# CameronDiao/MolCLR

Hardware: AMD Instinct MI355X
Metric: contrastive pre-train molecules/sec at batch 512, 1/2/4/8 MI355X; HBM GB/s on scatter_add (higher is better)
Workload: dtype f32; 1 GPU; c2: GIN 5x300 feat 512, batch 512/GPU, 10-50 atom graphs; model=gin 5x300 feat 512, global_batch=512, per_gpu_batch=512, mean_nodes_per_view=15278, mean_edges_per_view=25094, parallelism=dp1, views=one paired encoder pass, per-view BatchNorm statistics, augment=host: pre-built resident batch pairs

## Files before the change

molclr_amd/csrc/gemm.hip:

```cpp
#include "mfma.h"

#include <stdlib.h>

#include <type_traits>

namespace {

using namespace molclr;

constexpr int LDK = BK + 4;
constexpr int RPAD = 4;

template <bool KMAJOR, int ROWS>
struct Image {
  static constexpr int FLOATS = KMAJOR ? BK * (ROWS + RPAD) : ROWS * LDK;
};

template <bool KMAJOR, int ROWS, int T>
struct Stager {
  static constexpr int ITEMS = ROWS * BK / 4;
  static constexpr int PER_THREAD = (ITEMS + T - 1) / T;
  float4 r[PER_THREAD];
  uint32_t ok;

// ... 425 lines not shown
      }
    }
  };

  const int nsteps = kt_end - kt_beg;
  auto kof = [&](int step) { return (int64_t)(kt_beg + step) * BK; };
  constexpr int CSN = CS == 1 ? SA::PER : CS == 2 ? SB::PER : 1;
  float4 cs[CSN];
#pragma unroll
  for (int j = 0; j < CSN; ++j) cs[j] = make_float4(0.f, 0.f, 0.f, 0.f);
  if (nsteps > 0) {
    sa0.load(kof(0), K, ta);
    sb0.load(kof(0), K, tb);
    if (nsteps > 1) {
      sa1.load(kof(1), K, ta);
      sb1.load(kof(1), K, tb);
    }
    if constexpr (CS) sa0.colsum_add(cs, ta);
    sa0.store(buf0, ta);
    sb0.store(buf0 + AI, tb);
    __syncthreads();
  }
  int i = 0;
  for (; i + 2 <= nsteps; i += 2) {
    if (i + 2 < nsteps) {
      sa0.load(kof(i + 2), K, ta);
      sb0.load(kof(i + 2), K, tb);
    }
    compute(buf0);
    if constexpr (CS) sa1.colsum_add(cs, ta);
    sa1.store(buf1, ta);
    sb1.store(buf1 + AI, tb);
    __syncthreads();
    if (i + 3 < nsteps) {
      sa1.load(kof(i + 3), K, ta);
      sb1.load(kof(i + 3), K, tb);
    }
    compute(buf1);
    if constexpr (CS) {
      if (i + 2 < nsteps) sa0.colsum_add(cs, ta);
    }
    sa0.store(buf0, ta);
    sb0.store(buf0 + AI, tb);
    __syncthreads();
  }
  if (i < nsteps) compute(buf0);

  if constexpr (CS) {
    if (n0 == 0 && colsum != nullptr) {
      constexpr int RB = BM / 4;
      float4 v = cs[0];
#pragma unroll
      for (int j = 1; j < CSN; ++j) v = f4add(v, cs[j]);
      __syncthreads();
      float4* red = reinterpret_cast<float4*>(lds);
      red[tid] = v;
      __syncthreads();
      if (tid < RB) {
        float4 t4 = red[tid];
        for (int q = 1; q < T / RB; ++q) t4 = f4add(t4, red[tid + q * RB]);
        const float e[4] = {t4.x, t4.y, t4.z, t4.w};
        float* o = SPLIT ? colsum + (int64_t)blockIdx.y * M : colsum;
        for (int j = 0; j < 4; ++j) {
          const int64_t m = m0 + 4 * tid + j;
          if (m < M) o[m] = (!SPLIT && accumulate) ? o[m] + e[j] : e[j];
        }
      }
    }
  }

  float* Cout = SPLIT ? C + (int64_t)blockIdx.y * M * N : C;
  const int64_t ldo = SPLIT ? N : ldc;
  constexpr int WR = 32 * TM, WC = 32 * TN;
  static_assert(4 * WR * WC * (int)sizeof(float) <= (int)sizeof(lds), "epilogue tile > LDS");
  const bool vec = ((ldo & 3) == 0) && ((reinterpret_cast<uintptr_t>(Cout) & 15) == 0) &&
                   (SPLIT || EPI != MOLCLR_EPI_RELU_MASK ||
                    (((ldaux & 3) == 0) && (reinterpret_cast<uintptr_t>(aux) & 15) == 0)) &&
                   (SPLIT || (EPI != MOLCLR_EPI_BIAS && EPI != MOLCLR_EPI_BIAS_RELU) ||
                    (reinterpret_cast<uintptr_t>(bias) & 15) == 0);
  if (vec) {
    __syncthreads();
    float* tw = reinterpret_cast<float*>(lds) + wave * WR * WC;
#pragma unroll
    for (int a = 0; a < TM; ++a)
#pragma unroll
      for (int b = 0; b < TN; ++b)
#pragma unroll
        for (int r = 0; r < 16; ++r)
          tw[(a * 32 + (r & 3) + 8 * (r >> 2) + 4 * lh) * WC + b * 32 + li] =
              acc[a][b][r] + acl[a][b][r];
    __syncthreads();
    constexpr int C4 = WC / 4;
    const int64_t mw = m0 + wm * WR, nw = n0 + wn * WC;
#pragma unroll
    for (int it = 0; it < WR * C4 / 64; ++it) {
      const int idx = it * 64 + lane;
      const int row = idx / C4, c4 = idx - row * C4;
      const int64_t m = mw + row, n = nw + 4 * c4;
      if (m >= M || n >= N) continue;
      float4 v = *reinterpret_cast<const float4*>(tw + row * WC + 4 * c4);
      float* o = Cout + m * ldo + n;
      if (n + 4 <= N) {
        if (!SPLIT) {
          if (EPI == MOLCLR_EPI_BIAS || EPI == MOLCLR_EPI_BIAS_RELU) {
            const float4 bv = *reinterpret_cast<const float4*>(bias + n);
            v = f4add(v, bv);
            if (EPI == MOLCLR_EPI_BIAS_RELU)
              v = make_float4(fmaxf(v.x, 0.f), fmaxf(v.y, 0.f), fmaxf(v.z, 0.f), fmaxf(v.w, 0.f));
          }
          if (EPI == MOLCLR_EPI_RELU_MASK) {
            const float4 x = *reinterpret_cast<const float4*>(aux + m * ldaux + n);
            v = make_float4(x.x > 0.f ? v.x : 0.f, x.y > 0.f ? v.y : 0.f, x.z > 0.f ? v.z : 0.f,
                            x.w > 0.f ? v.w : 0.f);
          }
          if (accumulate) v = f4add(v, *reinterpret_cast<const float4*>(o));
        }
        *reinterpret_cast<float4*>(o) = v;
      } else {
        const float e[4] = {v.x, v.y, v.z, v.w};
        for (int j = 0; j < 4 && n + j < N; ++j) {
          float x = e[j];
          if (!SPLIT) {
            if (EPI == MOLCLR_EPI_BIAS) x = x + bias[n + j];
            if (EPI == MOLCLR_EPI_BIAS_RELU) x = fmaxf(x + bias[n + j], 0.f);
            if (EPI == MOLCLR_EPI_RELU_MASK) x = aux[m * ldaux + n + j] > 0.f ? x : 0.f;
            if (accumulate) x += o[j];
          }
          o[j] = x;
        }
      }
    }
    return;
  }
#pragma unroll
  for (int b = 0; b < TN; ++b) {
    const int64_t n = n0 + wn * TN * 32 + b * 32 + li;
    if (n >= N) continue;
    float bv = 0.f;
    if (!SPLIT && (EPI == MOLCLR_EPI_BIAS || EPI == MOLCLR_EPI_BIAS_RELU)) bv = bias[n];
#pragma unroll
    for (int a = 0; a < TM; ++a) {
#pragma unroll
      for (int r = 0; r < 16; ++r) {
        const int64_t m = m0 + wm * TM * 32 + a * 32 + (r & 3) + 8 * (r >> 2) + 4 * lh;
        if (m >= M) continue;
        float v = acc[a][b][r] + acl[a][b][r];
        if (!SPLIT) {
          if (EPI == MOLCLR_EPI_BIAS) v = v + bv;
          if (EPI == MOLCLR_EPI_BIAS_RELU) v = fmaxf(v + bv, 0.f);
          if (EPI == MOLCLR_EPI_RELU_MASK) v = aux[m * ldaux + n] > 0.f ? v : 0.f;
          if (accumulate) v += Cout[m * ldo + n];
        }
        Cout[m * ldo + n] = v;
      }
    }
  }
}

constexpr int kQ6Waves = 4;
constexpr int kQ6BM = 32 * kQ6Waves;
constexpr int64_t kQ6MaxK = 1024;

template <int BN, int T, int NP = 3>
struct QStageB {
  static constexpr int UNITS = NP * BN * 4;
  static constexpr int PER = (UNITS + T - 1) / T;
  u32x4 r[PER];
  int goff[PER];
  __device__ __forceinline__ void init(int64_t n0, int64_t npad, int64_t kp, int t) {
#pragma unroll
    for (int j = 0; j < PER; ++j) {
      const int u = t + j * T;
      const int pl = u / (BN * 4), rem = u % (BN * 4);
      int64_t row = n0 + (rem >> 2);
      row = row < npad ? row : npad - 1;
      goff[j] = (UNITS % T && u >= UNITS) ? 0 : (int)((pl * npad + row) * kp + 8 * (rem & 3));
    }
  }
  __device__ __forceinline__ void load(const uint16_t* __restrict__ Bp, int64_t k0, int t) {
#pragma unroll
    for (int j = 0; j < PER; ++j) {
      if (j == PER - 1 && UNITS % T && t + j * T >= UNITS) continue;
      r[j] = *reinterpret_cast<const u32x4*>(Bp + goff[j] + k0);
    }
  }
  __device__ __forceinline__ void store(uint16_t* __restrict__ img, int t) const {
#pragma unroll
    for (int j = 0; j < PER; ++j) {
      const int u = t + j * T;
      if (j == PER - 1 && UNITS % T && u >= UNITS) continue;
      const int pl = u / (BN * 4), rem = u % (BN * 4);
      *reinterpret_cast<u32x4*>(img + pl * BN * XK + xoff(rem >> 2, rem & 3)) = r[j];
    }
  }
};

template <int BN, int NP>
__device__ __forceinline__ void q6_dma_b(const uint16_t* __restrict__ Bp, int64_t n0, int64_t npad,
                                         int64_t kp, int64_t k0, uint16_t* img, int wm, int lane) {
  constexpr int RPB = BN / 16, CH = NP * RPB, PERW = (CH + kQ6Waves - 1) / kQ6Waves;
  static_assert(BN % 16 == 0, "q6 DMA: 16-row chunks");
#pragma unroll
  for (int qq = 0; qq < PERW; ++qq) {
    const int q = wm + kQ6Waves * qq;
    if (CH % kQ6Waves && q >= CH) break;
    const int pl = q / RPB, row = (q % RPB) * 16 + (lane >> 2), c = lane & 3;
    int64_t gr = n0 + row;
    gr = gr < npad ? gr : npad - 1;
    __builtin_amdgcn_global_load_lds(
        (gbl_as_ptr)(Bp + (pl * npad + gr) * kp + k0 + 8 * (c ^ ((row >> 2) & 3))),
        (lds_as_ptr)(img + (pl * BN + (q % RPB) * 16) * XK), 16, 0, 0);
  }
}

template <int TN, int EPI, int KG, bool MASK, int H3 = 0>
__global__ __launch_bounds__(64 * kQ6Waves * KG) __attribute__((amdgpu_waves_per_eu(2))) void k_gemm_q6(
    const float* __restrict__ A, const uint16_t* __restrict__ Bp, float* __restrict__ C,
    int64_t M, int64_t N, int64_t K, int64_t lda, int64_t kp, int64_t npad, int64_t ldc,
    const float* __restrict__ bias, const float* __restrict__ aux, int64_t ldaux,
    int accumulate, const float* __restrict__ amax, const float* __restrict__ bmax,
    float* __restrict__ cmax, float* __restrict__ crow, float* __restrict__ amax_out,
    int arow_parts, uint32_t* __restrict__ bits_out, const uint32_t* __restrict__ bits_in,
    int64_t bits_ld) {
  constexpr int T = 64 * kQ6Waves;
  constexpr int BN = 32 * TN;
  constexpr int NP = H3 ? 2 : 3;
  constexpr int BI = NP * BN * XK;
  constexpr int EPI_ELEMS = kQ6Waves * 32 * 32 * 2;
  constexpr int L0 = KG == 1 ? (BI > EPI_ELEMS ? BI : EPI_ELEMS) : KG * 2 * BI;
  static_assert(KG == 1 || (kQ6Waves * 32 * BN * (int)sizeof(float) <=
                            KG * 2 * BI * (int)sizeof(uint16_t)),
                "group sums exceed the LDS images");
  __shared__ __attribute__((aligned(16))) uint16_t lds[L0];
  __shared__ __attribute__((aligned(16))) uint16_t lds_b1[KG == 1 ? BI : 8];

  const int tid = threadIdx.x;
  const int lane = tid & 63;
  const int wave = __builtin_amdgcn_readfirstlane(tid >> 6);
  const int grp = wave / kQ6Waves, wm = wave % kQ6Waves, gt = tid - grp * T;
  const int li = lane & 31, lh = lane >> 5;

  const int ntn = (int)((N + BN - 1) / BN);
  const int ntm = (int)((M + kQ6BM - 1) / kQ6BM);
  const int tile = xcd_remap(blockIdx.x, ntm * ntn);
  const int64_t m0 = (int64_t)(tile / ntn) * kQ6BM;
  const int64_t n0 = (int64_t)(tile % ntn) * BN;

  constexpr bool HAS_BIAS = EPI == MOLCLR_EPI_BIAS || EPI == MOLCLR_EPI_BIAS_RELU;
  constexpr int BVN = HAS_BIAS ? TN : 1, MWN = EPI == MOLCLR_EPI_RELU_MASK ? TN : 1;
  float4 bvq[BVN];
  uint32_t mwq[MWN][4];
  if (grp == 0) {
    const int c4l = lane & 7;
    if constexpr (HAS_BIAS) {
#pragma unroll
      for (int b = 0; b < TN; ++b) {
        const int64_t n = n0 + 32 * b + 4 * c4l;
        bvq[b] = (n + 4 <= N && (reinterpret_cast<uintptr_t>(bias) & 15) == 0)
                     ? *reinterpret_cast<const float4*>(bias + n) : f4zero();
      }
    }
    if constexpr (EPI == MOLCLR_EPI_RELU_MASK) {
      if (bits_in != nullptr) {
#pragma unroll
        for (int b = 0; b < TN; ++b)
#pragma unroll
          for (int it = 0; it < 4; ++it) {
            int64_t m = m0 + 32 * wm + 8 * it + (lane >> 3);
            m = m < M ? m : M - 1;
            int64_t nb = n0 + 32 * b;
            nb = nb < N ? nb : 0;
            mwq[b][it] = bits_in[(nb >> 5) * bits_ld + m];
          }
      }
    }
  }

  int64_t arow_i = m0 + 32 * wm + li;
  arow_i = arow_i < M ? arow_i : M - 1;
  const float* __restrict__ arow = A + arow_i * lda;
  const int nsteps = (int)(kp / BK);
  const int rounds = (nsteps + KG - 1) / KG;
  auto kb = [&](int r) {
    const int st = grp + KG * r;
    return (int64_t)(st < nsteps ? st : nsteps - 1) * BK;
  };
  auto load_a = [&](int r, float4(&v)[4]) {
    r = r < rounds ? r : rounds - 1;
    const int64_t k = (int64_t)(grp + KG * r) * BK + 16 * lh;
#pragma unroll
    for (int j = 0; j < 4; ++j) {
      int64_t kj = k + 4 * j;
      if constexpr (MASK) kj = kj < K - 4 ? kj : K - 4;
      v[j] = *reinterpret_cast<const float4*>(arow + kj);
    }
  };

  f32x16 acc[TN];
#pragma unroll
  for (int b = 0; b < TN; ++b)
#pragma unroll
    for (int r = 0; r < 16; ++r) acc[b][r] = 0.f;

  int sha = 0;
  if constexpr (H3 == 1) sha = h3_shift(amax);
  if constexpr (H3 == 2) {
// ... 2079 lines not shown
                         a.K, a.lda, a.ldb, npad, a.ldc, a.bias, a.aux, a.ldaux, a.accumulate,
                         a.amax, a.bmax, a.cmax, a.crow, a.amax_out, a.arow_parts, a.bits_out,
                         a.bits_in, a.bits_ld, ntn, groups);
  else if (wv == 16)
    molclr::launch_timed(molclr::kTimeGemm, (k_gemm_bsn<EPI, H3, 19, false, 16, 64>),
                         dim3((unsigned)(ntn * groups)), dim3(1024), 0, s, a.A, a.Bp, a.C, a.M, a.N,
                         a.K, a.lda, a.ldb, npad, a.ldc, a.bias, a.aux, a.ldaux, a.accumulate,
                         a.amax, a.bmax, a.cmax, a.crow, a.amax_out, a.arow_parts, a.bits_out,
                         a.bits_in, a.bits_ld, ntn, groups);
  else
    molclr::launch_timed(molclr::kTimeGemm, (k_gemm_bsn<EPI, H3, 19, false, 12, 64>),
                         dim3((unsigned)(ntn * groups)), dim3(768), 0, s, a.A, a.Bp, a.C, a.M, a.N,
                         a.K, a.lda, a.ldb, npad, a.ldc, a.bias, a.aux, a.ldaux, a.accumulate,
                         a.amax, a.bmax, a.cmax, a.crow, a.amax_out, a.arow_parts, a.bits_out,
                         a.bits_in, a.bits_ld, ntn, groups);
}
template <int H3>
int dispatch_bs64(int epi, const Args& a, int64_t npad, hipStream_t s) {
  switch (epi) {
    case MOLCLR_EPI_NONE: launch_bs64<MOLCLR_EPI_NONE, H3>(a, npad, s); return 0;
    case MOLCLR_EPI_BIAS: launch_bs64<MOLCLR_EPI_BIAS, H3>(a, npad, s); return 0;
    case MOLCLR_EPI_BIAS_RELU: launch_bs64<MOLCLR_EPI_BIAS_RELU, H3>(a, npad, s); return 0;
    case MOLCLR_EPI_RELU_MASK: launch_bs64<MOLCLR_EPI_RELU_MASK, H3>(a, npad, s); return 0;
    default: return -1;
  }
}
int64_t crow_parts(int64_t N) { return N > 320 ? (N + kBN - 1) / kBN : q6_col_tiles(N); }

int run_q6(const Args& a, int64_t npad, int epi, hipStream_t s, int h3 = 0) {
  if (h3 != 0 && use_bs(a, npad, epi, h3)) {
    const int rc = h3 == 2 ? dispatch_bs<2>(epi, a, npad, s) : dispatch_bs<1>(epi, a, npad, s);
    if (rc) {
      molclr::set_error("gemm_f32_h3: no bs kernel for epilogue %d", epi);
      return MOLCLR_ERR_UNSUPPORTED;
    }
    MOLCLR_LAUNCHED();
    return MOLCLR_OK;
  }
  if (h3 != 0 && use_bs64(a, npad, epi, h3)) {
    const int rc = h3 == 2 ? dispatch_bs64<2>(epi, a, npad, s) : dispatch_bs64<1>(epi, a, npad, s);
    if (rc) {
      molclr::set_error("gemm_f32_h3: no bs64 kernel for epilogue %d", epi);
      return MOLCLR_ERR_UNSUPPORTED;
    }
    MOLCLR_LAUNCHED();
    return MOLCLR_OK;
  }
  if (g_bs_force >= 2) {
    molclr::set_error("gemm_f32_h3_impl: the bs kernel does not take this product");
    return MOLCLR_ERR_UNSUPPORTED;
  }
  if (a.crow != nullptr && crow_parts(a.N) > q6_col_tiles(a.N)) {
    const int64_t w = q6_col_tiles(a.N);
    const hipError_t e = molclr::zero_async(a.crow + w * a.M,
                                            (size_t)(crow_parts(a.N) - w) * a.M * sizeof(float), s);
    if (e != hipSuccess) return (int)e;
  }
  const int rc = h3 == 2   ? dispatch_q6_tn<2>(epi, a, npad, s)
                 : h3 == 1 ? dispatch_q6_tn<1>(epi, a, npad, s)
                           : dispatch_q6_tn<0>(epi, a, npad, s);
  if (rc) {
    molclr::set_error("gemm_f32_bplanes: no q6 kernel for epilogue %d", epi);
    return MOLCLR_ERR_UNSUPPORTED;
  }
  MOLCLR_LAUNCHED();
  return MOLCLR_OK;
}

struct W6Plan {
  int tn, splits, kps, kg;
  int64_t ntiles;
};
W6Plan w6_plan(int64_t M, int64_t N, int64_t K, int kg) {
  W6Plan p;
  p.tn = wide_tn(N);
  p.kg = kg;
  p.ntiles = ((M + kW6BM - 1) / kW6BM) * ((N + 32 * p.tn - 1) / (32 * p.tn));
  const int64_t nk = (K + BK - 1) / BK;
  int64_t s = (512 / p.kg) / p.ntiles;
  if (s > nk / (4 * p.kg)) s = nk / (4 * p.kg);
  if (s < 1) s = 1;
  p.kps = (int)((nk + s - 1) / s);
  p.splits = (int)((nk + p.kps - 1) / p.kps);
  return p;
}
bool w6_shape_ok(int64_t M, int64_t N, int64_t K) {
  return M % 4 == 0 && N % 4 == 0 && K >= 1024 && M * N < (1ll << 28);
}
size_t w6_ws_bytes(int64_t M, int64_t N, int64_t K, bool colsum) {
  size_t need = 0;
  for (int kg = 1; kg <= 2; ++kg)
    for (int tr = 0; tr < 2; ++tr) {
      const W6Plan p = tr ? w6_plan(N, M, K, kg) : w6_plan(M, N, K, kg);
      const size_t b = (size_t)p.splits * (M * N + (colsum ? M : 0)) * sizeof(float) + 256;
      need = b > need ? b : need;
    }
  return need;
}

template <int TN, int KG, bool H3>
void launch_w6_kg(const W6Plan& p, hipStream_t s, const float* A, const float* B, float* part,
                  int64_t M, int64_t N, int64_t K, int64_t lda, int64_t ldb, float* cs_part,
                  const float* amax, const float* bmax, bool cs_b) {
  const dim3 grid((unsigned)(p.ntiles * p.splits));
  if (cs_part && cs_b)
    molclr::launch_timed(molclr::kTimeGemm, (k_gemm_w6<TN, 2, KG, H3>), grid, dim3(256 * KG), 0,
                         s, A, B, part, M, N, K, lda, ldb, p.kps, p.splits, cs_part, amax, bmax);
  else if (cs_part)
    molclr::launch_timed(molclr::kTimeGemm, (k_gemm_w6<TN, 1, KG, H3>), grid, dim3(256 * KG), 0,
                         s, A, B, part, M, N, K, lda, ldb, p.kps, p.splits, cs_part, amax, bmax);
  else
    molclr::launch_timed(molclr::kTimeGemm, (k_gemm_w6<TN, 0, KG, H3>), grid, dim3(256 * KG),
                         0, s, A, B, part, M, N, K, lda, ldb, p.kps, p.splits, cs_part, amax, bmax);
}
template <int TN, bool H3>
void launch_w6(const W6Plan& p, hipStream_t s, const float* A, const float* B, float* part,
               int64_t M, int64_t N, int64_t K, int64_t lda, int64_t ldb, float* cs_part,
               const float* amax, const float* bmax, bool cs_b = false) {
  if (p.kg == 2)
    launch_w6_kg<TN, 2, H3>(p, s, A, B, part, M, N, K, lda, ldb, cs_part, amax, bmax, cs_b);
  else
    launch_w6_kg<TN, 1, H3>(p, s, A, B, part, M, N, K, lda, ldb, cs_part, amax, bmax, cs_b);
}

int run_w6(const float* A, const float* B, float* C, float* colsum, int64_t M, int64_t N,
           int64_t K, int64_t lda, int64_t ldb, int64_t ldc, int accumulate, void* ws,
           size_t ws_bytes, hipStream_t s, int kg = 2, const float* amax = nullptr,
           const float* bmax = nullptr) {
  const W6Plan p = w6_plan(M, N, K, kg);
  MOLCLR_REQUIRE_WS(ws_bytes, w6_ws_bytes(M, N, K, colsum != nullptr));
  float* part = static_cast<float*>(ws);
  float* cs_part = colsum ? part + (size_t)p.splits * M * N : nullptr;
  if (amax) {
    if (p.tn == 5) launch_w6<5, true>(p, s, A, B, part, M, N, K, lda, ldb, cs_part, amax, bmax);
    else if (p.tn == 4) launch_w6<4, true>(p, s, A, B, part, M, N, K, lda, ldb, cs_part, amax, bmax);
    else launch_w6<2, true>(p, s, A, B, part, M, N, K, lda, ldb, cs_part, amax, bmax);
  } else {
    if (p.tn == 5) launch_w6<5, false>(p, s, A, B, part, M, N, K, lda, ldb, cs_part, amax, bmax);
    else if (p.tn == 4) launch_w6<4, false>(p, s, A, B, part, M, N, K, lda, ldb, cs_part, amax, bmax);
    else launch_w6<2, false>(p, s, A, B, part, M, N, K, lda, ldb, cs_part, amax, bmax);
  }
  const float* no_f = nullptr;
  molclr::launch_timed(molclr::kTimeGemm, k_splitk_reduce<MOLCLR_EPI_NONE>,
                       dim3((unsigned)molclr::ceil_div(M * N, 256)), dim3(256), 0, s,
                       static_cast<const float*>(part), p.splits, M, N, C, ldc, no_f, no_f,
                       (int64_t)0, accumulate, static_cast<const float*>(cs_part), p.splits, colsum);
  MOLCLR_LAUNCHED();
  return MOLCLR_OK;
}

int64_t planes_npad(int64_t N) { return (N + kPlanesRowPad - 1) / kPlanesRowPad * kPlanesRowPad; }
int64_t planes_kp(int64_t K) { return (K + BK - 1) / BK * BK; }

int run_gemm(const Args& a0, int impl, bool bp, int a_kmajor, int b_kmajor, int epilogue,
             void* workspace, size_t workspace_bytes, hipStream_t s) {
  const int64_t M = a0.M, N = a0.N, K = a0.K;
  int64_t tiles = tiles_for(impl, M, N, a_kmajor, b_kmajor);
  MOLCLR_REQUIRE(tiles < (1ll << 31), "gemm_f32: too many tiles");
  int sp = pick_splits(impl, M, N, K, a_kmajor, b_kmajor);
  const size_t cs_floats = a0.colsum ? (size_t)M : 0;
  if (sp > 1 && workspace_bytes < (size_t)sp * (M * N + cs_floats) * sizeof(float)) sp = 1;
  Args a = a0;
  a.impl = impl;
  int rc;
  if (sp == 1) {
    rc = bp ? dispatch_bplanes<false>(impl, a_kmajor, epilogue, dim3((unsigned)tiles), s, a)
            : dispatch<false>(a_kmajor != 0, b_kmajor != 0, epilogue, dim3((unsigned)tiles), s, a);
  } else {
    int64_t nk = (K + BK - 1) / BK;
    int kps = (int)((nk + sp - 1) / sp);
    sp = (int)((nk + kps - 1) / kps);
    float* partial = (float*)workspace;
    float* cs_partial = a.colsum ? partial + (size_t)sp * M * N : nullptr;
    Args ap = a;
    ap.C = partial;
    ap.colsum = cs_partial;
    ap.ldc = N;
    ap.bias = nullptr;
    ap.aux = nullptr;
    ap.ldaux = 0;
    ap.kps = kps;
    ap.accumulate = 0;
    rc = bp ? dispatch_bplanes<true>(impl, a_kmajor, MOLCLR_EPI_NONE, dim3((unsigned)tiles, sp), s, ap)
            : dispatch<true>(a_kmajor != 0, b_kmajor != 0, MOLCLR_EPI_NONE,
                             dim3((unsigned)tiles, sp), s, ap);
    if (rc == 0) {
      dim3 g((unsigned)molclr::ceil_div(M * N, 256));
      float* C = a.C;
      const int64_t ldc = a.ldc, ldaux = a.ldaux;
      const float *bias = a.bias, *aux = a.aux;
      const int accumulate = a.accumulate;
      switch (epilogue) {
        case MOLCLR_EPI_NONE:
          molclr::launch_timed(molclr::kTimeGemm, k_splitk_reduce<MOLCLR_EPI_NONE>, g, dim3(256), 0, s,
                               partial, sp, M, N, C, ldc, bias, aux, ldaux, accumulate, cs_partial, sp, a.colsum);
          break;
        case MOLCLR_EPI_BIAS:
          molclr::launch_timed(molclr::kTimeGemm, k_splitk_reduce<MOLCLR_EPI_BIAS>, g, dim3(256), 0, s,
                               partial, sp, M, N, C, ldc, bias, aux, ldaux, accumulate, cs_partial, sp, a.colsum);
          break;
        case MOLCLR_EPI_BIAS_RELU:
          molclr::launch_timed(molclr::kTimeGemm, k_splitk_reduce<MOLCLR_EPI_BIAS_RELU>, g, dim3(256), 0,
                               s, partial, sp, M, N, C, ldc, bias, aux, ldaux, accumulate, cs_partial, sp, a.colsum);
          break;
        default:
          molclr::launch_timed(molclr::kTimeGemm, k_splitk_reduce<MOLCLR_EPI_RELU_MASK>, g, dim3(256), 0,
                               s, partial, sp, M, N, C, ldc, bias, aux, ldaux, accumulate, cs_partial, sp, a.colsum);
      }
    }
  }
  if (rc != 0) {
    molclr::set_error("gemm_f32: no kernel for this layout");
    return MOLCLR_ERR_UNSUPPORTED;
  }
  MOLCLR_LAUNCHED();
  return MOLCLR_OK;
}

}

void molclr_splitk_reduce_none(const float* partial, int splits, int64_t M, int64_t N, float* C,
                               int64_t ldc, int accumulate, const float* cs_partial,
                               int cs_splits, float* colsum, hipStream_t s) {
  const float* no_f = nullptr;
  molclr::launch_timed(molclr::kTimeGemm, k_splitk_reduce<MOLCLR_EPI_NONE>,
                       dim3((unsigned)molclr::ceil_div(M * N > M ? M * N : M, 256)), dim3(256), 0,
                       s, partial, splits, M, N, C, ldc, no_f, no_f, (int64_t)0, accumulate,
                       cs_partial, cs_splits, colsum);
}

MOLCLR_API size_t molclr_gemm_f32_workspace_bytes(int64_t M, int64_t N, int64_t K) {
  int sp = pick_splits(0, M, N, K);
  for (int impl = 5; impl <= 8; ++impl) {
    const int s2 = pick_splits(impl, M, N, K);
    sp = s2 > sp ? s2 : sp;
  }
  const int s3 = pick_splits(5, M, N, K, 1, 1);
  sp = s3 > sp ? s3 : sp;
  size_t need = sp > 1 ? (size_t)sp * M * N * sizeof(float) + 256 : 0;
  if (w6_shape_ok(M, N, K)) {
    const size_t w6 = w6_ws_bytes(M, N, K, false);
    need = w6 > need ? w6 : need;
  }
  return need;
}

MOLCLR_API int molclr_gemm_f32_impl(const float* A, const float* B, float* C, int64_t M, int64_t N,
                                    int64_t K, int64_t lda, int64_t ldb, int64_t ldc, int a_kmajor,
                                    int b_kmajor, int epilogue_flags, const float* bias,
                                    const float* aux, int64_t ldaux, void* workspace,
                                    size_t workspace_bytes, molclr_stream_t stream, int impl_req) {
  const int accumulate = (epilogue_flags & MOLCLR_EPI_ACCUMULATE) ? 1 : 0;
  const int epilogue = epilogue_flags & ~MOLCLR_EPI_ACCUMULATE;
  MOLCLR_REQUIRE(impl_req == -1 || impl_req == 0 || impl_req == 5 || impl_req == 6,
                 "gemm_f32: impl %d (-1 automatic, 0, 5, 6)", impl_req);
  MOLCLR_REQUIRE(M >= 0 && N >= 0 && K >= 0, "gemm_f32: negative size");
  MOLCLR_REQUIRE(epilogue >= MOLCLR_EPI_NONE && epilogue <= MOLCLR_EPI_RELU_MASK,
                 "gemm_f32: bad epilogue %d", epilogue);
  MOLCLR_REQUIRE((epilogue != MOLCLR_EPI_BIAS && epilogue != MOLCLR_EPI_BIAS_RELU) || bias,
                 "gemm_f32: bias epilogue needs bias");
  MOLCLR_REQUIRE(epilogue != MOLCLR_EPI_RELU_MASK || aux, "gemm_f32: relu-mask epilogue needs aux");
  MOLCLR_REQUIRE(a_kmajor || (K % 4 == 0 && lda % 4 == 0),
                 "gemm_f32: A with K contiguous needs K (%lld) and lda multiples of 4", (long long)K);
  MOLCLR_REQUIRE(b_kmajor || (K % 4 == 0 && ldb % 4 == 0),
                 "gemm_f32: B with K contiguous needs K (%lld) and ldb multiples of 4", (long long)K);
  MOLCLR_REQUIRE(ldc >= N && (a_kmajor ? lda >= M : lda >= K) && (b_kmajor ? ldb >= N : ldb >= K),
                 "gemm_f32: leading dimension too small");
  if (M == 0 || N == 0) return MOLCLR_OK;
  hipStream_t s = molclr::as_stream(stream);
  if (K == 0) {
    molclr::set_error("gemm_f32: K == 0 unsupported");
    return MOLCLR_ERR_UNSUPPORTED;
  }
  const int impl = impl_for(M, N, lda, ldb, a_kmajor, b_kmajor, impl_req);
  if (impl_req == -1 && impl == 5 && a_kmajor && b_kmajor && epilogue == MOLCLR_EPI_NONE &&
      w6_shape_ok(M, N, K) && lda % 4 == 0 && ldb % 4 == 0 &&
      workspace_bytes >= w6_ws_bytes(M, N, K, false))
    return run_w6(A, B, C, nullptr, M, N, K, lda, ldb, ldc, accumulate, workspace,
                  workspace_bytes, s);
  Args a{A, B, C, M, N, K, lda, ldb, ldc, bias, aux, ldaux, 0, accumulate, impl};
  return run_gemm(a, impl, false, a_kmajor, b_kmajor, epilogue, workspace, workspace_bytes, s);
}

MOLCLR_API int molclr_gemm_f32(const float* A, const float* B, float* C, int64_t M, int64_t N,
                               int64_t K, int64_t lda, int64_t ldb, int64_t ldc, int a_kmajor,
                               int b_kmajor, int epilogue_flags, const float* bias, const float* aux,
                               int64_t ldaux, void* workspace, size_t workspace_bytes,
                               molclr_stream_t stream) {
  return molclr_gemm_f32_impl(A, B, C, M, N, K, lda, ldb, ldc, a_kmajor, b_kmajor, epilogue_flags,
                              bias, aux, ldaux, workspace, workspace_bytes, stream, -1);
}

MOLCLR_API size_t molclr_bplanes_bytes(int64_t N, int64_t K) {
  return (size_t)3 * planes_npad(N) * planes_kp(K) * sizeof(uint16_t);
}

MOLCLR_API int molclr_bplanes_make(const float* B, int64_t N, int64_t K, int64_t ldb, int b_kmajor,
                                   uint16_t* planes, molclr_stream_t stream) {
  MOLCLR_REQUIRE(N > 0 && K > 0 && B && planes, "bplanes_make: empty or null operand");
  MOLCLR_REQUIRE(b_kmajor ? ldb >= N : ldb >= K, "bplanes_make: leading dimension too small");
  PlanesJobs jobs{};
  jobs.j[0] = PlanesJob{B, planes, N, K, ldb, planes_npad(N), planes_kp(K), b_kmajor};
  hipLaunchKernelGGL(k_planes_make_tiled<false>, dim3((unsigned)planes_tiled_blocks(jobs.j[0]), 1),
                     dim3(256), 0, molclr::as_stream(stream), jobs);
  MOLCLR_LAUNCHED();
  return MOLCLR_OK;
}

MOLCLR_API int molclr_bplanes_make_batch(int count, const float* const* B, const int64_t* N,
                                         const int64_t* K, const int64_t* ldb,
                                         const int* b_kmajor, uint16_t* const* planes,
                                         molclr_stream_t stream) {
  MOLCLR_REQUIRE(count >= 0 && (count == 0 || (B && N && K && ldb && b_kmajor && planes)),
                 "bplanes_make_batch: null arrays");
  for (int base = 0; base < count; base += kPlanesBatch) {
    PlanesJobs jobs{};
    const int n = count - base < kPlanesBatch ? count - base : kPlanesBatch;
    int64_t most = 0;
    for (int i = 0; i < n; ++i) {
      const int q = base + i;
      MOLCLR_REQUIRE(N[q] > 0 && K[q] > 0 && B[q] && planes[q],
                     "bplanes_make_batch: job %d empty or null", q);
      MOLCLR_REQUIRE(b_kmajor[q] ? ldb[q] >= N[q] : ldb[q] >= K[q],
                     "bplanes_make_batch: job %d leading dimension too small", q);
      jobs.j[i] = PlanesJob{B[q], planes[q], N[q], K[q], ldb[q], planes_npad(N[q]), planes_kp(K[q]),
                            b_kmajor[q]};
      const int64_t e = planes_tiled_blocks(jobs.j[i]);
      most = e > most ? e : most;
    }
    hipLaunchKernelGGL(k_planes_make_tiled<false>, dim3((unsigned)most, (unsigned)n), dim3(256), 0,
                       molclr::as_stream(stream), jobs);
  }
  MOLCLR_LAUNCHED();
  return MOLCLR_OK;
}

MOLCLR_API int molclr_gemm_f32_bplanes_tile(const float* A, const uint16_t* planes, float* C,
                                            int64_t M, int64_t N, int64_t K, int64_t lda,
                                            int64_t ldc, int a_kmajor, int epilogue_flags,
                                            const float* bias, const float* aux, int64_t ldaux,
                                            void* workspace, size_t workspace_bytes,
                                            molclr_stream_t stream, int tile) {
  const int accumulate = (epilogue_flags & MOLCLR_EPI_ACCUMULATE) ? 1 : 0;
  const int epilogue = epilogue_flags & ~MOLCLR_EPI_ACCUMULATE;
  MOLCLR_REQUIRE(tile == 0 || (tile >= 5 && tile <= 9),
                 "gemm_f32_bplanes: tile %d (0 automatic, 5..9)", tile);
  MOLCLR_REQUIRE(M >= 0 && N >= 0 && K >= 0, "gemm_f32_bplanes: negative size");
  MOLCLR_REQUIRE(epilogue >= MOLCLR_EPI_NONE && epilogue <= MOLCLR_EPI_RELU_MASK,
                 "gemm_f32_bplanes: bad epilogue %d", epilogue);
  MOLCLR_REQUIRE((epilogue != MOLCLR_EPI_BIAS && epilogue != MOLCLR_EPI_BIAS_RELU) || bias,
                 "gemm_f32_bplanes: bias epilogue needs bias");
  MOLCLR_REQUIRE(epilogue != MOLCLR_EPI_RELU_MASK || aux,
                 "gemm_f32_bplanes: relu-mask epilogue needs aux");
  MOLCLR_REQUIRE(a_kmajor ? (M % 4 == 0 && lda % 4 == 0 && lda >= M)
                          : (K % 4 == 0 && lda % 4 == 0 && lda >= K),
                 "gemm_f32_bplanes: A needs 4-aligned rows (K-major) or K (K contiguous)");
  MOLCLR_REQUIRE(ldc >= N, "gemm_f32_bplanes: ldc < N");
  if (M == 0 || N == 0) return MOLCLR_OK;
  MOLCLR_REQUIRE(K > 0 && A && planes && C, "gemm_f32_bplanes: null operand or K == 0");
  const int64_t npad = planes_npad(N), kp = planes_kp(K);
  int impl = tile;
  if (impl == 0) impl = (!a_kmajor && q6_blocks(M, N) >= 128) ? 9 : (N >= 512 ? 7 : 5);
  if (impl == 9 && (a_kmajor || K > kQ6MaxK || 3 * npad * kp >= (1ll << 31) ||
                    q6_blocks(M, N) >= (1ll << 31)))
    impl = N >= 512 ? 7 : 5;
  if ((impl == 6 || impl == 8) && a_kmajor) impl = 5;
  Args a{A, nullptr, C, M, N, K, lda, kp, ldc, bias, aux, ldaux, 0, accumulate, impl};
  a.Bp = planes;
  a.bps = npad * kp;
  if (impl == 9) return run_q6(a, npad, epilogue, molclr::as_stream(stream));
  return run_gemm(a, impl, true, a_kmajor, 0, epilogue, workspace, workspace_bytes,
                  molclr::as_stream(stream));
}

MOLCLR_API int molclr_gemm_f32_bplanes_max(const float* A, const uint16_t* planes, float* C,
                                           int64_t M, int64_t N, int64_t K, int64_t lda,
                                           int64_t ldc, int epilogue_flags, const float* bias,
                                           const float* aux, int64_t ldaux, float* amax_out,
                                           float* cmax, float* crow, uint32_t* relu_bits,
                                           void* workspace, size_t workspace_bytes,
                                           molclr_stream_t stream) {
  const int accumulate = (epilogue_flags & MOLCLR_EPI_ACCUMULATE) ? 1 : 0;
  const int epilogue = epilogue_flags & ~MOLCLR_EPI_ACCUMULATE;
  MOLCLR_REQUIRE(M >= 0 && N >= 0 && K >= 0, "gemm_f32_bplanes_max: negative size");
  MOLCLR_REQUIRE(epilogue >= MOLCLR_EPI_NONE && epilogue <= MOLCLR_EPI_RELU_MASK,
                 "gemm_f32_bplanes_max: bad epilogue %d", epilogue);
  MOLCLR_REQUIRE((epilogue != MOLCLR_EPI_BIAS && epilogue != MOLCLR_EPI_BIAS_RELU) || bias,
                 "gemm_f32_bplanes_max: bias epilogue needs bias");
  MOLCLR_REQUIRE(epilogue != MOLCLR_EPI_RELU_MASK || aux,
                 "gemm_f32_bplanes_max: relu-mask epilogue needs aux");
  MOLCLR_REQUIRE(K % 4 == 0 && lda % 4 == 0 && lda >= K && ldc >= N && K <= kQ6MaxK,
                 "gemm_f32_bplanes_max: K (<= %lld) and lda multiples of 4, lda >= K, ldc >= N",
                 (long long)kQ6MaxK);
  if (M == 0 || N == 0) return MOLCLR_OK;
  MOLCLR_REQUIRE(K > 0 && A && planes && C, "gemm_f32_bplanes_max: null operand or K == 0");
  const int64_t npad = planes_npad(N), kp = planes_kp(K);
  MOLCLR_REQUIRE(3 * npad * kp < (1ll << 31) && q6_blocks(M, N) < (1ll << 31),
                 "gemm_f32_bplanes_max: too large");
  hipStream_t s = molclr::as_stream(stream);
  if (q6_blocks(M, N) < 128) {
    MOLCLR_TRY_RC(molclr_gemm_f32_bplanes(A, planes, C, M, N, K, lda, ldc, 0, epilogue_flags, bias,
                                          aux, ldaux, workspace, workspace_bytes, stream));
    if (amax_out) MOLCLR_TRY_RC(molclr_absmax_f32(A, M, K, lda, amax_out, 1, stream));
    if (relu_bits) {
      const int64_t words = (N + 31) / 32;
      hipLaunchKernelGGL(k_relu_bits, dim3((unsigned)molclr::ceil_div(M * words, 256)), dim3(256),
                         0, s, C, M, N, ldc, relu_bits, words);
    }
    if (crow || cmax) {
      float* rows = crow;
      if (!rows) {
        MOLCLR_TRY_RC(molclr_absmax_f32(C, M, N, ldc, cmax, 1, stream));
        return MOLCLR_OK;
      }
      int64_t blocks = molclr::ceil_div(M, 32);
      blocks = blocks < 1 ? 1 : blocks > 2048 ? 2048 : blocks;
      hipLaunchKernelGGL(k_absmax_rows, dim3((unsigned)blocks), dim3(256), 0, s, C, M, N, ldc, rows,
                         cmax);
      for (int64_t p = 1; p < crow_parts(N); ++p)
        (void)molclr::copy_async(rows + p * M, rows, (size_t)M * sizeof(float), s);
    }
    MOLCLR_LAUNCHED();
    return MOLCLR_OK;
  }
  Args a{A, nullptr, C, M, N, K, lda, kp, ldc, bias, aux, ldaux, 0, accumulate, 9};
  a.Bp = planes;
  a.bps = npad * kp;
  a.cmax = cmax;
  a.crow = crow;
  a.amax_out = amax_out;
  a.bits_out = relu_bits;
  a.bits_ld = M;
  return run_q6(a, npad, epilogue, s, 0);
}

MOLCLR_API int64_t molclr_gemm_row_parts(int64_t N) { return crow_parts(N); }

MOLCLR_API int molclr_gemm_f32_bplanes(const float* A, const uint16_t* planes, float* C, int64_t M,
                                       int64_t N, int64_t K, int64_t lda, int64_t ldc,
                                       int a_kmajor, int epilogue_flags, const float* bias,
                                       const float* aux, int64_t ldaux, void* workspace,
                                       size_t workspace_bytes, molclr_stream_t stream) {
  return molclr_gemm_f32_bplanes_tile(A, planes, C, M, N, K, lda, ldc, a_kmajor, epilogue_flags,
                                      bias, aux, ldaux, workspace, workspace_bytes, stream, 0);
}

size_t molclr_colsum_ws(int64_t rows, int64_t cols);

MOLCLR_API size_t molclr_linear_wgrad_workspace_bytes(int64_t rows, int64_t n_out, int64_t n_in) {
  const int64_t M = n_out, N = n_in, K = rows;
  size_t need = molclr_gemm_f32_workspace_bytes(M, N, K);
  const int sp = pick_splits(5, M, N, K, 1, 1);
  const size_t fused = sp > 1 ? (size_t)sp * (M * N + M) * sizeof(float) + 256 : 0;
  const size_t cs = molclr_colsum_ws(rows, n_out);
  need = fused > need ? fused : need;
  if (M % 4 == 0 && N % 4 == 0 && M * N < (1ll << 28)) {
    const size_t w6 = w6_ws_bytes(M, N, K, true);
    need = w6 > need ? w6 : need;
  }
  return cs > need ? cs : need;
}

MOLCLR_API int molclr_linear_wgrad_groups(const float* dy, const float* x, float* dW, float* db,
                                          int64_t rows, int64_t n_out, int64_t n_in, int64_t ld_dy,
                                          int64_t ld_x, int accumulate, void* workspace,
                                          size_t workspace_bytes, molclr_stream_t stream,
                                          int groups) {
  MOLCLR_REQUIRE(groups == 1 || groups == 2, "linear_wgrad: groups must be 1 or 2");
  MOLCLR_REQUIRE(rows >= 0 && n_out > 0 && n_in > 0, "linear_wgrad: bad sizes");
  MOLCLR_REQUIRE(dy && x && dW, "linear_wgrad: null pointer");
  MOLCLR_REQUIRE(ld_dy >= n_out && ld_x >= n_in, "linear_wgrad: leading dimension too small");
  MOLCLR_REQUIRE(!db || (n_out % 4 == 0 && ld_dy % 4 == 0),
                 "linear_wgrad: db needs n_out and ld_dy multiples of 4");
  MOLCLR_REQUIRE_WS(workspace_bytes, molclr_linear_wgrad_workspace_bytes(rows, n_out, n_in));
  const int flags = accumulate ? MOLCLR_EPI_ACCUMULATE : 0;
  if (rows == 0) {
    if (!accumulate) {
      (void)molclr::zero_async(dW, (size_t)n_out * n_in * sizeof(float), molclr::as_stream(stream));
      if (db) (void)molclr::zero_async(db, (size_t)n_out * sizeof(float), molclr::as_stream(stream));
    }
    MOLCLR_LAUNCHED();
    return MOLCLR_OK;
  }
  if (w6_shape_ok(n_out, n_in, rows) && ld_dy % 4 == 0 && ld_x % 4 == 0)
    return run_w6(dy, x, dW, db, n_out, n_in, rows, ld_dy, ld_x, n_in, accumulate, workspace,
                  workspace_bytes, molclr::as_stream(stream), groups);
  if (!db || impl_for(n_out, n_in, ld_dy, ld_x, 1, 1, -1) != 5) {
    int rc = molclr_gemm_f32(dy, x, dW, n_out, n_in, rows, ld_dy, ld_x, n_in, 1, 1, flags,
                             nullptr, nullptr, 0, workspace, workspace_bytes, stream);
    if (rc || !db) return rc;
    return molclr_colsum_f32(dy, db, rows, n_out, ld_dy, accumulate, workspace, workspace_bytes,
                             stream);
  }
  Args a{dy, x, dW, n_out, n_in, rows, ld_dy, ld_x, n_in, nullptr, nullptr, 0, 0, accumulate, 5};
  a.colsum = db;
  return run_gemm(a, 5, false, 1, 1, MOLCLR_EPI_NONE, workspace, workspace_bytes,
                  molclr::as_stream(stream));
}

MOLCLR_API int molclr_linear_wgrad(const float* dy, const float* x, float* dW, float* db,
                                   int64_t rows, int64_t n_out, int64_t n_in, int64_t ld_dy,
                                   int64_t ld_x, int accumulate, void* workspace,
                                   size_t workspace_bytes, molclr_stream_t stream) {
  return molclr_linear_wgrad_groups(dy, x, dW, db, rows, n_out, n_in, ld_dy, ld_x, accumulate,
                                    workspace, workspace_bytes, stream, 2);
}

MOLCLR_API int molclr_absmax_f32(const float* x, int64_t rows, int64_t cols, int64_t ld,
                                 float* slot, int accumulate, molclr_stream_t stream) {
  MOLCLR_REQUIRE(rows >= 0 && cols >= 0 && ld >= cols && slot, "absmax_f32: bad arguments");
  hipStream_t s = molclr::as_stream(stream);
  if (!accumulate) (void)molclr::zero_async(slot, kMaxSlotFloats * sizeof(float), s);
  if (rows > 0 && cols > 0) {
    MOLCLR_REQUIRE(x, "absmax_f32: null x");
    int64_t blocks = ld == cols ? molclr::ceil_div(rows * cols, 256 * 16) : rows;
    blocks = blocks < 1 ? 1 : blocks > 1024 ? 1024 : blocks;
    hipLaunchKernelGGL(k_absmax, dim3((unsigned)blocks), dim3(256), 0, s, x, rows, cols, ld, slot);
  }
  MOLCLR_LAUNCHED();
  return MOLCLR_OK;
}

MOLCLR_API int molclr_absmax_rows_f32(const float* x, int64_t rows, int64_t cols, int64_t ld,
// ... 288 lines not shown
```

Baseline: 194,300 molecules/s.

## Add in-block split-K small-M GEMM kernel reducing K-parts through LDS

Adds a new 512-thread GEMM kernel for small-M shapes (M up to 2048, K up to 1024) that splits the K loop across four wave groups inside one block. Each group double-buffers its own LDS images, and the partial sums are reduced in LDS and written through a fused bias/relu/mask epilogue. This replaces the separate split-K partial buffer and reduce kernel launch with a single launch. The kernel is enabled by default (env toggle), and is routed to from both the plain and bplanes entry points when impl 5 is selected. The cost is more threads per small tile, an LDS reduction step, and idle wave groups whenever the split count is below four.

```diff
diff --git a/molclr_amd/csrc/gemm.hip b/molclr_amd/csrc/gemm.hip
--- a/molclr_amd/csrc/gemm.hip
+++ b/molclr_amd/csrc/gemm.hip
@@ -601,6 +601,173 @@
           if (accumulate) v += Cout[m * ldo + n];
         }
         Cout[m * ldo + n] = v;
+      }
+    }
+  }
+}
+
+constexpr int64_t kS6MaxM = 2048;
+constexpr int64_t kS6MaxK = 1024;
+constexpr int kS6Parts = 4;
+
+template <int BMODE, int EPI>
+__global__ __launch_bounds__(512) void k_gemm_s6(
+    const float* __restrict__ A, const float* __restrict__ Bf, const uint16_t* __restrict__ Bp,
+    float* __restrict__ C, int64_t M, int64_t N, int64_t K, int64_t lda, int64_t ldb,
+    int64_t bplane_stride, int64_t ldc, const float* __restrict__ bias,
+    const float* __restrict__ aux, int64_t ldaux, int accumulate, int splits,
+    int ktiles_per_split) {
+  constexpr int T = 512, BM = 32, BN = 64;
+  constexpr int NI = kS6Parts;
+  constexpr int TI = T / NI;
+  constexpr int AI = 3 * BM * XK, BI = 3 * BN * XK;
+  constexpr int STEP = NI * (AI + BI);
+  static_assert(NI * BM * BN * (int)sizeof(float) <= 2 * STEP * (int)sizeof(uint16_t),
+                "the K-part sums exceed the LDS images");
+  __shared__ __attribute__((aligned(16))) uint16_t lds[2 * STEP];
+
+  const int tid = threadIdx.x;
+  const int lane = tid & 63, wave = tid >> 6;
+  const int nt = wave & 1, kq = wave >> 1;
+  const int li = lane & 31, lh = lane >> 5;
+  const int hi = tid / TI, ti = tid - hi * TI;
+
+  const int ntn = (int)((N + BN - 1) / BN);
+  const int ntm = (int)((M + BM - 1) / BM);
+  const int tile = xcd_remap(blockIdx.x, ntm * ntn);
+  const int64_t m0 = (int64_t)(tile / ntn) * BM;
+  const int64_t n0 = (int64_t)(tile % ntn) * BN;
+
+  const int nk_total = (int)((K + BK - 1) / BK);
+  auto tiles_of = [&](int h) {
+    if (h >= splits) return 0;
+    const int left = nk_total - h * ktiles_per_split;
+    return left < 0 ? 0 : left < ktiles_per_split ? left : ktiles_per_split;
+  };
+  const int nstage = tiles_of(hi);
+  const int ncomp = tiles_of(kq);
+  const int nsteps = ktiles_per_split;
+
+  f32x16 acc, acl;
+#pragma unroll
+  for (int r = 0; r < 16; ++r) acc[r] = acl[r] = 0.f;
+
+  using SA = PStageK<BM, TI>;
+  using SB = typename PStageSel<BMODE, BN, TI>::type;
+  SA sa0, sa1;
+  SB sb0, sb1;
+  sa0.init(A, lda, m0, M, ti);
+  if constexpr (BMODE == 2) sb0.init(Bp, ldb, bplane_stride, n0, ti);
+  else sb0.init(Bf, ldb, n0, N, ti);
+  sa1 = sa0;
+  sb1 = sb0;
+  uint16_t* buf0 = lds;
+  uint16_t* buf1 = lds + STEP;
+  const int io = hi * (AI + BI);
+
+  auto kof = [&](int step) { return ((int64_t)hi * ktiles_per_split + step) * BK; };
+  auto load = [&](SA& sa, SB& sb, int step) {
+    if (step < nstage) {
+      sa.load(kof(step), K, ti);
+      sb.load(kof(step), K, ti);
+    }
+  };
+  auto compute = [&](const uint16_t* buf, int step) {
+    if (step >= ncomp) return;
+    const uint16_t* As = buf + kq * (AI + BI);
+    const uint16_t* Bs = As + AI;
+    const int bro = nt * 32;
+#pragma unroll
+    for (int ks = 0; ks < 2; ++ks) {
+      bf16x8 bh, bm, bl;
+      if constexpr (BMODE == 1) {
+        bh = kmfrag<BN>(Bs, bro, ks, lane);
+        bm = kmfrag<BN>(Bs + BN * XK, bro, ks, lane);
+        bl = kmfrag<BN>(Bs + 2 * BN * XK, bro, ks, lane);
+      } else {
+        bh = xfrag(Bs, bro + li, ks * 2 + lh);
+        bm = xfrag(Bs + BN * XK, bro + li, ks * 2 + lh);
+        bl = xfrag(Bs + 2 * BN * XK, bro + li, ks * 2 + lh);
+      }
+      const bf16x8 ah = xfrag(As, li, ks * 2 + lh);
+      const bf16x8 am = xfrag(As + BM * XK, li, ks * 2 + lh);
+      const bf16x8 al = xfrag(As + 2 * BM * XK, li, ks * 2 + lh);
+      acl = __builtin_amdgcn_mfma_f32_32x32x16_bf16(ah, bl, acl, 0, 0, 0);
+      acl = __builtin_amdgcn_mfma_f32_32x32x16_bf16(al, bh, acl, 0, 0, 0);
+      acl = __builtin_amdgcn_mfma_f32_32x32x16_bf16(am, bm, acl, 0, 0, 0);
+      acl = __builtin_amdgcn_mfma_f32_32x32x16_bf16(ah, bm, acl, 0, 0, 0);
+      acl = __builtin_amdgcn_mfma_f32_32x32x16_bf16(am, bh, acl, 0, 0, 0);
+      acc = __builtin_amdgcn_mfma_f32_32x32x16_bf16(ah, bh, acc, 0, 0, 0);
+    }
+  };
+
+  if (nsteps > 0) {
+    load(sa0, sb0, 0);
+    load(sa1, sb1, 1);
+    sa0.store(buf0 + io, ti);
+    sb0.store(buf0 + io + AI, ti);
+    __syncthreads();
+  }
+  int i = 0;
+  for (; i + 2 <= nsteps; i += 2) {
+    load(sa0, sb0, i + 2);
+    compute(buf0, i);
+    sa1.store(buf1 + io, ti);
+    sb1.store(buf1 + io + AI, ti);
+    __syncthreads();
+    load(sa1, sb1, i + 3);
+    compute(buf1, i + 1);
+    sa0.store(buf0 + io, ti);
+    sb0.store(buf0 + io + AI, ti);
+    __syncthreads();
+  }
+  if (i < nsteps) compute(buf0, i);
+  __syncthreads();
+
+  float* red = reinterpret_cast<float*>(lds);
+#pragma unroll
+  for (int r = 0; r < 16; ++r)
+    red[(kq * BM + acc_row(r, lh)) * BN + nt * 32 + li] = acc[r] + acl[r];
+  __syncthreads();
+  const bool vec = ((ldc & 3) == 0) && ((reinterpret_cast<uintptr_t>(C) & 15) == 0) &&
+                   (EPI != MOLCLR_EPI_RELU_MASK ||
+                    (((ldaux & 3) == 0) && (reinterpret_cast<uintptr_t>(aux) & 15) == 0)) &&
+                   ((EPI != MOLCLR_EPI_BIAS && EPI != MOLCLR_EPI_BIAS_RELU) ||
+                    (reinterpret_cast<uintptr_t>(bias) & 15) == 0);
+  constexpr int C4 = BN / 4;
+  for (int idx = tid; idx < BM * C4; idx += T) {
+    const int row = idx / C4, c4 = idx - row * C4;
+    const int64_t m = m0 + row, n = n0 + 4 * c4;
+    if (m >= M || n >= N) continue;
+    float4 v = *reinterpret_cast<const float4*>(red + row * BN + 4 * c4);
+    if (splits > 1) {
+      v = f4add(make_float4(0.f, 0.f, 0.f, 0.f), v);
+      for (int q = 1; q < splits; ++q)
+        v = f4add(v, *reinterpret_cast<const float4*>(red + (q * BM + row) * BN + 4 * c4));
+    }
+    float* o = C + m * ldc + n;
+    if (vec && n + 4 <= N) {
+      if (EPI == MOLCLR_EPI_BIAS || EPI == MOLCLR_EPI_BIAS_RELU) {
+        v = f4add(v, *reinterpret_cast<const float4*>(bias + n));
+        if (EPI == MOLCLR_EPI_BIAS_RELU)
+          v = make_float4(fmaxf(v.x, 0.f), fmaxf(v.y, 0.f), fmaxf(v.z, 0.f), fmaxf(v.w, 0.f));
+      }
+      if (EPI == MOLCLR_EPI_RELU_MASK) {
+        const float4 x = *reinterpret_cast<const float4*>(aux + m * ldaux + n);
+        v = make_float4(x.x > 0.f ? v.x : 0.f, x.y > 0.f ? v.y : 0.f, x.z > 0.f ? v.z : 0.f,
+                        x.w > 0.f ? v.w : 0.f);
+      }
+      if (accumulate) v = f4add(v, *reinterpret_cast<const float4*>(o));
+      *reinterpret_cast<float4*>(o) = v;
+    } else {
+      const float e[4] = {v.x, v.y, v.z, v.w};
+      for (int j = 0; j < 4 && n + j < N; ++j) {
+        float x = e[j];
+        if (EPI == MOLCLR_EPI_BIAS) x = x + bias[n + j];
+        if (EPI == MOLCLR_EPI_BIAS_RELU) x = fmaxf(x + bias[n + j], 0.f);
+        if (EPI == MOLCLR_EPI_RELU_MASK) x = aux[m * ldaux + n + j] > 0.f ? x : 0.f;
+        if (accumulate) x += o[j];
+        o[j] = x;
       }
     }
   }
@@ -2986,6 +3153,57 @@
 int64_t planes_npad(int64_t N) { return (N + kPlanesRowPad - 1) / kPlanesRowPad * kPlanesRowPad; }
 int64_t planes_kp(int64_t K) { return (K + BK - 1) / BK * BK; }
 
+bool gemm_small() {
+  static const bool on = [] {
+    const char* e = getenv("MOLCLR_GEMM_SMALL");
+    return !(e != nullptr && e[0] == '0');
+  }();
+  return on;
+}
+void p6_parts(int impl, int64_t M, int64_t N, int64_t K, int b_kmajor, size_t workspace_bytes,
+              int* splits, int* kps) {
+  int sp = pick_splits(impl, M, N, K, 0, b_kmajor);
+  if (sp > 1 && workspace_bytes < (size_t)sp * M * N * sizeof(float)) sp = 1;
+  const int64_t nk = (K + BK - 1) / BK;
+  *kps = (int)((nk + sp - 1) / sp);
+  *splits = (int)((nk + *kps - 1) / *kps);
+}
+bool s6_shape_ok(int impl, int64_t M, int64_t N, int64_t K, int a_kmajor, int b_kmajor,
+                 int64_t ldb, size_t workspace_bytes) {
+  if (!gemm_small() || a_kmajor || M > kS6MaxM || K > kS6MaxK || K <= 0) return false;
+  if (b_kmajor && (N % 4 != 0 || ldb % 4 != 0)) return false;
+  if (((M + 31) / 32) * ((N + 63) / 64) >= (1ll << 31)) return false;
+  int sp, kps;
+  p6_parts(impl, M, N, K, b_kmajor, workspace_bytes, &sp, &kps);
+  return sp <= kS6Parts;
+}
+
+template <int BMODE, int EPI>
+void launch_s6(hipStream_t s, const Args& a, int splits, int kps) {
+  const int64_t tiles = ((a.M + 31) / 32) * ((a.N + 63) / 64);
+  molclr::launch_timed(molclr::kTimeGemm, (k_gemm_s6<BMODE, EPI>), dim3((unsigned)tiles),
+                       dim3(512), 0, s, a.A, a.B, a.Bp, a.C, a.M, a.N, a.K, a.lda, a.ldb, a.bps,
+                       a.ldc, a.bias, a.aux, a.ldaux, a.accumulate, splits, kps);
+}
+template <int BMODE>
+void launch_s6_epi(int epi, hipStream_t s, const Args& a, int splits, int kps) {
+  switch (epi) {
+    case MOLCLR_EPI_NONE: launch_s6<BMODE, MOLCLR_EPI_NONE>(s, a, splits, kps); break;
+    case MOLCLR_EPI_BIAS: launch_s6<BMODE, MOLCLR_EPI_BIAS>(s, a, splits, kps); break;
+    case MOLCLR_EPI_BIAS_RELU: launch_s6<BMODE, MOLCLR_EPI_BIAS_RELU>(s, a, splits, kps); break;
+    default: launch_s6<BMODE, MOLCLR_EPI_RELU_MASK>(s, a, splits, kps);
+  }
+}
+int run_s6(const Args& a, int impl, int bmode, int epi, size_t workspace_bytes, hipStream_t s) {
+  int sp, kps;
+  p6_parts(impl, a.M, a.N, a.K, bmode == 1, workspace_bytes, &sp, &kps);
+  if (bmode == 2) launch_s6_epi<2>(epi, s, a, sp, kps);
+  else if (bmode == 1) launch_s6_epi<1>(epi, s, a, sp, kps);
+  else launch_s6_epi<0>(epi, s, a, sp, kps);
+  MOLCLR_LAUNCHED();
+  return MOLCLR_OK;
+}
+
 int run_gemm(const Args& a0, int impl, bool bp, int a_kmajor, int b_kmajor, int epilogue,
              void* workspace, size_t workspace_bytes, hipStream_t s) {
   const int64_t M = a0.M, N = a0.N, K = a0.K;
@@ -3107,6 +3325,11 @@
     return MOLCLR_ERR_UNSUPPORTED;
   }
   const int impl = impl_for(M, N, lda, ldb, a_kmajor, b_kmajor, impl_req);
+  if (impl_req == -1 && impl == 5 &&
+      s6_shape_ok(impl, M, N, K, a_kmajor, b_kmajor, ldb, workspace_bytes)) {
+    Args a{A, B, C, M, N, K, lda, ldb, ldc, bias, aux, ldaux, 0, accumulate, impl};
+    return run_s6(a, impl, b_kmajor ? 1 : 0, epilogue, workspace_bytes, s);
+  }
   if (impl_req == -1 && impl == 5 && a_kmajor && b_kmajor && epilogue == MOLCLR_EPI_NONE &&
       w6_shape_ok(M, N, K) && lda % 4 == 0 && ldb % 4 == 0 &&
       workspace_bytes >= w6_ws_bytes(M, N, K, false))
@@ -3203,6 +3426,8 @@
   a.Bp = planes;
   a.bps = npad * kp;
   if (impl == 9) return run_q6(a, npad, epilogue, molclr::as_stream(stream));
+  if (tile == 0 && s6_shape_ok(impl, M, N, K, a_kmajor, 0, kp, workspace_bytes))
+    return run_s6(a, impl, 2, epilogue, workspace_bytes, molclr::as_stream(stream));
   return run_gemm(a, impl, true, a_kmajor, 0, epilogue, workspace, workspace_bytes,
                   molclr::as_stream(stream));
 }
```

Result: no change. 195,200 molecules/s (median of 6 runs) (+0.4%).
